# awkrail/svpc

Measured on AMD Instinct MI355X. Metric: train steps/sec (vivt, batch=16, clip_seq=12), higher is better.
Workload: dtype bf16x3; 1 GPU; MODEL_TYPE=vivt train step: N=16 videos/GPU x S=12 clips x Lv=100 frames x F=3072, Lt=22, D=768, H=12, L=6 (enc+step-enc+dec), V=951, A=384, E=10; dropout .1/.1/.4; fwd+bwd+allreduce+clip+BertAdam; mode=bf16x3, global_batch=16, parallelism=dp1, launch=hipGraph replay, gpus_requested=1

## Files before the change

### include/svpc_hip.h

```cpp
#ifndef SVPC_HIP_H
#define SVPC_HIP_H
#include <stddef.h>
#ifdef __cplusplus
extern "C" {
#endif

typedef struct ihipStream_t* svpc_stream_t;
typedef unsigned long long svpc_u64;

#define SVPC_ACT_NONE 0
#define SVPC_ACT_RELU 1
#define SVPC_ACT_GELU 2
#define SVPC_ACT_SIGMOID 3

const char* svpc_last_error(void);
int svpc_abi_version(void);

int svpc_ln_fwd(const float* x, const int* src_rows, const float* res, const float* gamma, const float* beta, float* y,
                float* mean, float* rstd, int R, int D, float eps, float p_pre, unsigned site_pre, float p_post,
                unsigned site_post, const svpc_u64* seed, const float* add1, int mod1, const float* add2, const int* idx2,
                svpc_stream_t stream);
int svpc_ln_fwd_t(const void* x, int x_dt, const int* src_rows, const void* res, const float* gamma, const float* beta, void* y,
                  int y_dt, float* mean, float* rstd, int R, int D, float eps, float p_pre, unsigned site_pre, float p_post,
                  unsigned site_post, const svpc_u64* seed, const float* add1, int mod1, const float* add2, const int* idx2,
// ... 9 lines not shown
int svpc_ln_fwd_s(const void* x, int x_dt, int ldx, int lox, const int* src_rows, const void* res, int ldr, int lor, const float* gamma,
                  const float* beta, void* y, int y_dt, int ldy, int loy, float* mean, float* rstd, int R, int D, float eps, float p_pre,
                  unsigned site_pre, float p_post, unsigned site_post, const svpc_u64* seed, const float* add1, int mod1,
                  const float* add2, const int* idx2, svpc_stream_t stream);
int svpc_ln_bwd_rows_s(const void* dy, const void* x, int x_dt, int ldx, int y_dt, const int* src_rows, const void* res, int ldr,
                       const float* gamma, const float* mean, const float* rstd, void* dh, void* dx, float* partial, int R, int D,
                       float p_pre, unsigned site_pre, float p_post, unsigned site_post, const svpc_u64* seed, svpc_stream_t stream);
int svpc_bucket_colsum_t(const void* x, int x_dt, int ldx, const int* idx, int R, int C, int K, float* out, int accumulate,
                         float* workspace, svpc_stream_t stream);
typedef struct svpc_finalize_entry { const float* partial; float* out0; float* out1; int groups, ncols, split; } svpc_finalize_entry;
int svpc_colsum_partial_t(const void* x, int x_dt, int ldx, int R, int C, float* partial, svpc_stream_t stream);
typedef struct svpc_colsum_entry { const void* x; float* partial; int dt, ldx, R, C; } svpc_colsum_entry;
int svpc_multi_colsum(const svpc_colsum_entry* entries, int n, svpc_stream_t stream);
int svpc_multi_finalize_max(void);
int svpc_multi_finalize(const svpc_finalize_entry* entries, int n, svpc_stream_t stream);
int svpc_ln_bwd_groups(int R);
int svpc_ln_param_only_groups(int R);
int svpc_ln_param_grads_g(const float* partial, int groups, int D, float* dgamma, float* dbeta, int accumulate, svpc_stream_t stream);
int svpc_ln_bwd(const float* dy, const float* x, const int* src_rows, const float* res, const float* gamma,
                const float* mean, const float* rstd, float* dh, float* dx, float* dgamma, float* dbeta, int accumulate,
                float* workspace, int R, int D, float p_pre, unsigned site_pre, float p_post, unsigned site_post,
                const svpc_u64* seed, svpc_stream_t stream);
int svpc_colsum_chunks(int R);
int svpc_bucket_colsum(const float* x, int ldx, const int* idx, int R, int C, int K, float* out, int accumulate,
                       float* workspace, svpc_stream_t stream);

int svpc_gemm_f32(const float* A, int lda, int a_kc, const float* B, int ldb, int b_kc, float* C, int ldc, float* Z, int M, int N,
                  int K, const float* bias, int act, float p_drop, unsigned site, const svpc_u64* seed, int accumulate,
                  float* workspace, size_t workspace_bytes, svpc_stream_t stream);
int svpc_gemm_bf16(const float* A, int lda, int a_kc, const float* B, int ldb, int b_kc, float* C, int ldc, float* Z, int M, int N,
                   int K, const float* bias, int act, float p_drop, unsigned site, const svpc_u64* seed, int accumulate,
                   float* workspace, size_t workspace_bytes, svpc_stream_t stream);
int svpc_gemm_mx(const void* A, int a_dt, int lda, int a_kc, const void* B, int b_dt, int ldb, int b_kc, void* C, int c_dt, int ldc,
                 void* Z, int M, int N, int K, const float* bias, int act, float p_drop, unsigned site, const svpc_u64* seed,
                 int accumulate, float* workspace, size_t workspace_bytes, svpc_stream_t stream);
int svpc_gemm_glds_supported(int a_kc, int b_kc, int lda, int ldb, int M, int N, int K);
int svpc_gemm_glds(const void* A, int lda, int a_kc, const void* B, int ldb, int b_kc, void* C, int c_dt, int ldc, void* Z, int M, int N,
                   int K, const float* bias, int act, float p_drop, unsigned site, const svpc_u64* seed, int accumulate,
                   float* workspace, size_t workspace_bytes, svpc_stream_t stream);
int svpc_gemm_glds_r(const void* A, int lda, int a_kc, const void* B, int ldb, int b_kc, void* C, int c_dt, int ldc, void* Z, const void* R,
                     int M, int N, int K, const float* bias, int act, float p_drop, unsigned site, const svpc_u64* seed, int accumulate,
                     float* workspace, size_t workspace_bytes, svpc_stream_t stream);
int svpc_gemm_glds_rg(const void* A, int lda, int a_kc, const void* B, int ldb, int b_kc, void* C, int c_dt, int ldc, void* Z, const void* R,
                      const void* G, int gact, int M, int N, int K, const float* bias, int act, float p_drop, unsigned site,
                      const svpc_u64* seed, int accumulate, float* workspace, size_t workspace_bytes, svpc_stream_t stream);
int svpc_gemm_p8(const void* A, int lda, const void* B, int ldb, void* C, int ldc, void* Z, int M, int N, int K, const float* bias, int act,
                 svpc_stream_t stream);
int svpc_gemm_p8x3_supported(int lda, int a_lo, int ldb, int ldc, int c_lo, int ldz, int M, int N, int K);
int svpc_gemm_p8x3(const void* A, int lda, int a_lo, const void* B, int ldb, long long b_lo, void* C, int ldc, int c_lo, void* Z, int ldz,
                   int M, int N, int K, const float* bias, int act, svpc_stream_t stream);
int svpc_gemm_s4x3(const void* A, int lda, int a_lo, const void* B, int ldb, long long b_lo, void* C, int ldc, int c_lo, void* Z, int ldz,
                   int M, int N, int K, const float* bias, int act, svpc_stream_t stream);
int svpc_gemm_s4t_supported(int lda, int ldb, int ldc, int M, int N, int K);
int svpc_gemm_s4t(const void* A, int lda, const void* B, int ldb, void* C, int ldc, const void* R, int M, int N, int K, svpc_stream_t stream);
int svpc_gemm_p8t_supported(int lda, int ldb, int ldc, int M, int N, int K);
int svpc_gemm_p8t(const void* A, int lda, const void* B, int ldb, void* C, int ldc, const void* G, int gact, const void* R, int M, int N, int K,
                  svpc_stream_t stream);
int svpc_gemm_l32_supported(int a_kc, int b_kc, int lda, int ldb, int M, int N, int K);
int svpc_gemm_l32_preferred(int a_kc, int b_kc, int lda, int ldb, int M, int N, int K);
int svpc_gemm_l32(const float* A, int lda, int a_kc, const float* B, int ldb, int b_kc, float* C, int ldc, float* Z, int M, int N, int K,
                  const float* bias, int act, float p_drop, unsigned site, const svpc_u64* seed, int accumulate, float* workspace,
                  size_t workspace_bytes, svpc_stream_t stream);
int svpc_gemm_l32_r(const float* A, int lda, int a_kc, const float* B, int ldb, int b_kc, float* C, int ldc, float* Z, const float* R, int M,
                    int N, int K, const float* bias, int act, float p_drop, unsigned site, const svpc_u64* seed, int accumulate,
                    float* workspace, size_t workspace_bytes, svpc_stream_t stream);
int svpc_gemm_l32_rg(const float* A, int lda, int a_kc, const float* B, int ldb, int b_kc, float* C, int ldc, const float* R, const float* G,
                     int gact, int M, int N, int K, int accumulate, float* workspace, size_t workspace_bytes, svpc_stream_t stream);
int svpc_gemm_l32_x3(const float* A, int lda, int a_kc, const float* B, int ldb, int b_kc, float* C, int ldc, float* Z, const float* R, int M,
                     int N, int K, const float* bias, int act, float p_drop, unsigned site, const svpc_u64* seed, int accumulate,
                     float* workspace, size_t workspace_bytes, svpc_stream_t stream);
typedef struct svpc_gemm_problem { const float* A; const float* B; float* C; int M, N, K, lda, ldb, ldc; } svpc_gemm_problem;
int svpc_gemm_group(const svpc_gemm_problem* problems, int n, int a_kc, int b_kc, int accumulate, svpc_stream_t stream);
int svpc_gemm_group_x3(const svpc_gemm_problem* problems, int n, int a_kc, int b_kc, int accumulate, svpc_stream_t stream);
typedef struct svpc_wgrad_problem {
    const float* dz; const float* x; float* dw; float* db;
    int n_out, n_in, rows, ld_dz, ld_x, ld_dw;
} svpc_wgrad_problem;
int svpc_gemm_group_wgrad_max(void);
int svpc_gemm_group_wgrad_bf16_p8_ok(const void* problems, int n);
int svpc_gemm_group_wgrad_bf16_p8(const void* problems, int n, float* workspace, size_t workspace_bytes, svpc_stream_t stream);
int svpc_gemm_group_wgrad_bf16(const svpc_wgrad_problem* problems, int n, svpc_stream_t stream);
int svpc_gemm_group_wgrad_bf16_ws(const svpc_wgrad_problem* problems, int n, float* workspace, size_t workspace_bytes,
                                  svpc_stream_t stream);
int svpc_gemm_group_wgrad(const svpc_wgrad_problem* problems, int n, svpc_stream_t stream);
int svpc_act_bwd(const float* dy, const float* aux, float* dz, size_t n, int act, float p, unsigned site, const svpc_u64* seed,
                 svpc_stream_t stream);

int svpc_act_bwd_t(const void* dy, const void* aux, void* dz, int dt, size_t n, int act, float p, unsigned site, const svpc_u64* seed,
                   svpc_stream_t stream);

int svpc_attn_fwd(const float* Q, int ldq, const float* K, int ldk, const float* V, int ldv, float* O, int ldo, float* LSE,
                  const int* seq, int n_seq, int H, int dh, int max_q, int max_k, const float* key_mask, int causal, float scale,
                  float p_drop, unsigned site, const svpc_u64* seed, svpc_stream_t stream);
int svpc_attn_q1_fwd(const float* Q, int ldq, const float* K, int ldk, const float* V, int ldv, float* O, int ldo, float* LSE,
                     const int* seq, int n_seq, int H, int dh, int max_k, const float* key_mask, float scale, svpc_stream_t stream);
int svpc_attn_q1_ln_supported(int D, int dh, int n_keys, int ldq, int ldkv, int ldnew, int ldx, int ldo);
int svpc_attn_q1_ln_fwd(const float* Q, int ldq, float* K, float* V, int ldkv, int k_stride, int n_keys, const float* newK, const float* newV,
                        int ldnew, const float* X, int ldx, const float* gamma, const float* beta, float eps, float* O, int ldo, int T, int D,
                        int dh, float scale, svpc_stream_t stream);
int svpc_attn_q1_ln_idx_fwd(const float* Q, int ldq, float* K, float* V, int ldkv, int k_stride, int n_keys, const int* key_rows, int ld_rows,
                            int q_group, const float* newK, const float* newV, int ldnew, const float* X, int ldx, const float* gamma,
                            const float* beta, float eps, float* O, int ldo, int T, int D, int dh, float scale, svpc_stream_t stream);
int svpc_attn_bwd(const float* Q, int ldq, const float* K, int ldk, const float* V, int ldv, const float* O, int ldo,
                  const float* LSE, const float* dO, int lddo, float* dQ, int lddq, float* dK, int lddk, float* dV, int lddv,
                  float* delta, const int* seq, int n_seq, int H, int dh, int max_q, int max_k, const float* key_mask, int causal,
                  float scale, float p_drop, unsigned site, const svpc_u64* seed, svpc_stream_t stream);
// ... 203 lines not shown
```

### svpc_amd/csrc/gemm_common.h

```cpp
#pragma once
#include "common.h"

typedef float floatx16 __attribute__((ext_vector_type(16)));

struct Epi {
    const float* bias; int act; float p_drop; uint32_t site; const u64* seed; int accumulate;
    float* Z;
    const void* R;
    const void* G; int gact;
};

__device__ __forceinline__ void epilogue_store(float v, int row, int col, float* __restrict__ C, int ldc, const Epi& e,
                                               u64 seed, float inv_keep) {
    if (e.bias) v += e.bias[col];
    const size_t o = (size_t)row * ldc + col;
    if (e.Z) e.Z[o] = v;
    v = apply_act(v, e.act);
    if (e.p_drop > 0.f) v *= drop_scale(seed, e.site, o, e.p_drop, inv_keep);
    if (e.G) v *= act_grad_from_aux(reinterpret_cast<const float*>(e.G)[o], e.gact, false);
    if (e.accumulate) v += C[o];
    if (e.R) v += reinterpret_cast<const float*>(e.R)[o];
    C[o] = v;
}

// ... 67 lines not shown
    return (xcd < r ? xcd * (q + 1) : r * (q + 1) + (xcd - r) * q) + (orig >> 3);
}


template <typename TC>
__global__ __launch_bounds__(256) void splitk_reduce1_kernel(const float* __restrict__ slabs, int splitk, TC* __restrict__ C, int ldc,
                                                             int M, int N, Epi epi) {
    const size_t i = (size_t)blockIdx.x * 256 + threadIdx.x;
    if (i >= (size_t)M * N) return;
    const int row = (int)(i / N), col = (int)(i - (size_t)row * N);
    float s = 0.f;
    for (int k = 0; k < splitk; ++k) s += slabs[(size_t)k * M * N + i];
    const u64 seed = epi.p_drop > 0.f ? epi.seed[0] : 0ull;
    const float inv_keep = epi.p_drop > 0.f ? 1.0f / (1.0f - epi.p_drop) : 1.0f;
    epilogue_store_t<TC>(s, row, col, C, ldc, epi, seed, inv_keep);
}
template <typename TC>
__global__ __launch_bounds__(256) void splitk_reduce4_kernel(const float* __restrict__ slabs, int splitk, TC* __restrict__ C, int ldc,
                                                             int M, int N, Epi epi) {
    const size_t q = (size_t)blockIdx.x * 256 + threadIdx.x, nq = (size_t)M * N / 4;
    if (q >= nq) return;
    const size_t i = q * 4;
    const int row = (int)(i / N), col = (int)(i - (size_t)row * N);
    const float4* p = reinterpret_cast<const float4*>(slabs) + q;
    float4 s = make_float4(0.f, 0.f, 0.f, 0.f);
    int k = 0;
    for (; k + 4 <= splitk; k += 4) {
        const float4 a = p[(size_t)k * nq], b = p[(size_t)(k + 1) * nq], c = p[(size_t)(k + 2) * nq], d = p[(size_t)(k + 3) * nq];
        s.x += a.x; s.y += a.y; s.z += a.z; s.w += a.w;
        s.x += b.x; s.y += b.y; s.z += b.z; s.w += b.w;
        s.x += c.x; s.y += c.y; s.z += c.z; s.w += c.w;
        s.x += d.x; s.y += d.y; s.z += d.z; s.w += d.w;
    }
    for (; k < splitk; ++k) {
        const float4 a = p[(size_t)k * nq];
        s.x += a.x; s.y += a.y; s.z += a.z; s.w += a.w;
    }
    const u64 seed = epi.p_drop > 0.f ? epi.seed[0] : 0ull;
    const float inv_keep = epi.p_drop > 0.f ? 1.0f / (1.0f - epi.p_drop) : 1.0f;
    epilogue_store_t<TC>(s.x, row, col, C, ldc, epi, seed, inv_keep);
    epilogue_store_t<TC>(s.y, row, col + 1, C, ldc, epi, seed, inv_keep);
    epilogue_store_t<TC>(s.z, row, col + 2, C, ldc, epi, seed, inv_keep);
    epilogue_store_t<TC>(s.w, row, col + 3, C, ldc, epi, seed, inv_keep);
}
template <typename TC>
static inline void launch_splitk_reduce(const float* slabs, int splitk, TC* C, int ldc, int M, int N, const Epi& epi, hipStream_t stream) {
    const size_t n = (size_t)M * N;
    if (N % 4 == 0 && ((((uintptr_t)slabs) & 15) == 0))
        hipLaunchKernelGGL(splitk_reduce4_kernel<TC>, dim3((unsigned)((n / 4 + 255) / 256)), dim3(256), 0, stream, slabs, splitk, C, ldc, M, N,
                           epi);
    else
        hipLaunchKernelGGL(splitk_reduce1_kernel<TC>, dim3((unsigned)((n + 255) / 256)), dim3(256), 0, stream, slabs, splitk, C, ldc, M, N, epi);
}
```

### svpc_amd/csrc/gemm_s4t.hip

```cpp
#include "gemm_common.h"
#include <stdlib.h>

typedef __bf16 bf16x8 __attribute__((ext_vector_type(8)));
typedef float floatx4 __attribute__((ext_vector_type(4)));
typedef short short4s __attribute__((ext_vector_type(4)));
typedef const void __attribute__((address_space(1))) * s4t_gptr;
typedef void __attribute__((address_space(3))) * s4t_lptr;

constexpr int S4T_BK = 64;
constexpr int S4T_HALF = 128 * S4T_BK * 2;
constexpr int S4T_STAGE = 2 * S4T_HALF;

__device__ __forceinline__ bf16x8 s4t_frag_tr(const char* __restrict__ a) {
    typedef short4s __attribute__((address_space(3))) * lds_ptr;
    const short4s lo = __builtin_amdgcn_ds_read_tr16_b64_v4i16((lds_ptr)(a));
    const short4s hi = __builtin_amdgcn_ds_read_tr16_b64_v4i16((lds_ptr)(a + 4 * 256));
    union { short s[8]; bf16x8 v; } u;
    u.s[0] = lo[0]; u.s[1] = lo[1]; u.s[2] = lo[2]; u.s[3] = lo[3];
    u.s[4] = hi[0]; u.s[5] = hi[1]; u.s[6] = hi[2]; u.s[7] = hi[3];
    return u.v;
}

template <bool HASR, int NS>
__global__ __launch_bounds__(512, NS == 2 ? 2 : 1) void gemm_s4t_kernel(const __bf16* __restrict__ A, int lda, const __bf16* __restrict__ B, int ldb,
                                                                        __bf16* __restrict__ C, int ldc, const __bf16* __restrict__ R, int M,
                                                                        int N, int K, int tiles_m, int tiles_n, int remap) {
    __shared__ __attribute__((aligned(1024))) char smem[NS * S4T_STAGE];
    const int wg = remap ? xcd_remap(blockIdx.x, tiles_m * tiles_n) : (int)blockIdx.x;
    const int tm = wg / tiles_n, tn = wg - tm * tiles_n;
    const int m0 = tm * 128, n0 = tn * 128;
    const int nk = K / S4T_BK;
    const int lane = threadIdx.x & 63, wave = __builtin_amdgcn_readfirstlane(threadIdx.x >> 6);
    const int wr = wave >> 1, wc = wave & 1;

    const int sr = lane >> 2, sc = (lane & 3) ^ (((lane >> 5) & 1) << 1);
    const __bf16* const ga = A + (size_t)min(m0 + 16 * wave + sr, M - 1) * lda + 8 * sc;
    const __bf16* gb[2];
#pragma unroll
    for (int u = 0; u < 2; ++u) {
        const int kr = 8 * wave + 4 * u + (lane >> 4);
        const int fx = 2 * ((kr & 3) | ((kr >> 1) & 4));
        const int col = min(n0 + 8 * ((lane & 15) ^ fx), N - 8);
        gb[u] = B + (size_t)kr * ldb + col;
    }
    const size_t stepB = (size_t)S4T_BK * ldb;
#define S4T_ISSUE(t)                                                                                                              \
    do {                                                                                                                          \
        char* st_ = smem + ((t) % NS) * S4T_STAGE;                                                                                \
        const __bf16* sa_ = ga + (size_t)(t) * S4T_BK;                                                                            \
        __builtin_amdgcn_global_load_lds((s4t_gptr)(sa_), (s4t_lptr)(st_ + ((wave * 2) << 10)), 16, 0, 0);                        \
        __builtin_amdgcn_global_load_lds((s4t_gptr)(sa_ + 32), (s4t_lptr)(st_ + ((wave * 2 + 1) << 10)), 16, 0, 0);               \
        __builtin_amdgcn_global_load_lds((s4t_gptr)(gb[0] + (size_t)(t) * stepB), (s4t_lptr)(st_ + S4T_HALF + wave * 2048), 16, 0, 0);        \
        __builtin_amdgcn_global_load_lds((s4t_gptr)(gb[1] + (size_t)(t) * stepB), (s4t_lptr)(st_ + S4T_HALF + wave * 2048 + 1024), 16, 0, 0); \
    } while (0)
    const int fr_off = (lane & 15) * 64 + ((((lane >> 4) ^ (((lane >> 3) & 1) << 1))) << 4);
#define S4T_FRAGA(img, blk, kb) (*reinterpret_cast<const bf16x8*>((img) + (((blk) * 2 + (kb)) << 10) + fr_off))
    const int tg = lane >> 4, tq = (lane & 15) >> 2, tp = lane & 3;
    const int tfx = 2 * (tq + 4 * (tg & 1));
    const int tb_off = (8 * tg + tq) * 256 + ((tp & 1) << 3);
    const int tp1 = tp >> 1;
#define S4T_FRAGB(img, cb, kb) s4t_frag_tr((img) + (kb) * (32 * 256) + tb_off + (((((2 * (cb)) ^ tfx)) | tp1) << 4))

    floatx4 acc[2][4];
#pragma unroll
    for (int i = 0; i < 2; ++i)
#pragma unroll
        for (int j = 0; j < 4; ++j) acc[i][j] = floatx4{0.f, 0.f, 0.f, 0.f};

#pragma unroll
    for (int t = 0; t < NS - 1; ++t)
        if (t < nk) S4T_ISSUE(t);
    for (int t = 0; t < nk; ++t) {
        if (NS == 4 && t + 2 < nk) asm volatile("s_waitcnt vmcnt(8)" ::: "memory");
        else if (NS >= 3 && t + 1 < nk) asm volatile("s_waitcnt vmcnt(4)" ::: "memory");
        else asm volatile("s_waitcnt vmcnt(0)" ::: "memory");
        __builtin_amdgcn_s_barrier();
        __builtin_amdgcn_sched_barrier(0);
        if (t + NS - 1 < nk) S4T_ISSUE(t + NS - 1);
        const char* sa = smem + (t % NS) * S4T_STAGE;
        const char* sb = sa + S4T_HALF;
#pragma unroll
        for (int kb = 0; kb < 2; ++kb) {
            bf16x8 bfr[4], afr[2];
#pragma unroll
            for (int j = 0; j < 4; ++j) bfr[j] = S4T_FRAGB(sb, wc * 4 + j, kb);
#pragma unroll
            for (int i = 0; i < 2; ++i) afr[i] = S4T_FRAGA(sa, wr * 2 + i, kb);
#pragma unroll
            for (int i = 0; i < 2; ++i)
#pragma unroll
                for (int j = 0; j < 4; ++j) acc[i][j] = __builtin_amdgcn_mfma_f32_16x16x32_bf16(bfr[j], afr[i], acc[i][j], 0, 0, 0);
        }
    }
#undef S4T_ISSUE
#undef S4T_FRAGA
#undef S4T_FRAGB
    __syncthreads();
    char* wl = smem + wave * 8192;
    const int row0 = m0 + wr * 32, col0 = n0 + wc * 64;
    const int l15 = lane & 15, q = lane >> 4;
    const int c8 = lane & 7, cc = col0 + 8 * c8, r0 = lane >> 3;
    const bool col_ok = cc + 8 <= N;
    bf16x8 rv[HASR ? 4 : 1];
#pragma unroll
    for (int it = 0; it < 4; ++it) {
        const int r = it * 8 + r0;
        if (HASR && col_ok && row0 + r < M) rv[it] = *reinterpret_cast<const bf16x8*>(R + (size_t)(row0 + r) * ldc + cc);
    }
#pragma unroll
    for (int i = 0; i < 2; ++i) {
        const int r = i * 16 + l15;
#pragma unroll
        for (int j = 0; j < 4; ++j) {
            const int c16 = j * 4 + q;
            *reinterpret_cast<floatx4*>(wl + r * 256 + ((c16 ^ (r & 7)) << 4)) = acc[i][j];
        }
    }
#pragma unroll
    for (int it = 0; it < 4; ++it) {
        const int r = it * 8 + r0;
        const floatx4 v0 = *reinterpret_cast<const floatx4*>(wl + r * 256 + (((2 * c8) ^ (r & 7)) << 4));
        const floatx4 v1 = *reinterpret_cast<const floatx4*>(wl + r * 256 + (((2 * c8 + 1) ^ (r & 7)) << 4));
        float v[8] = {v0[0], v0[1], v0[2], v0[3], v1[0], v1[1], v1[2], v1[3]};
        if (col_ok && row0 + r < M) {
            const size_t o = (size_t)(row0 + r) * ldc + cc;
            if (HASR) {
#pragma unroll
                for (int j = 0; j < 8; ++j) v[j] += (float)rv[it][j];
            }
            bf16x8 ov;
#pragma unroll
            for (int j = 0; j < 8; ++j) ov[j] = (__bf16)v[j];
            *reinterpret_cast<bf16x8*>(C + o) = ov;
        }
    }
}

extern "C" {

int svpc_gemm_s4t_supported(int lda, int ldb, int ldc, int M, int N, int K) {
    if (M <= 0 || N < 8 || K < S4T_BK || K % S4T_BK != 0 || (N & 7) != 0) return 0;
    if ((lda & 7) || (ldb & 7) || (ldc & 7) || lda < K || ldb < N || ldc < N) return 0;
    return 1;
}

int svpc_gemm_s4t(const void* A, int lda, const void* B, int ldb, void* C, int ldc, const void* R, int M, int N, int K, hipStream_t stream) {
    if (M <= 0 || N <= 0) return 0;
    SVPC_REQUIRE(svpc_gemm_s4t_supported(lda, ldb, ldc, M, N, K) == 1 &&
                     ((((uintptr_t)A) | ((uintptr_t)B) | ((uintptr_t)C) | ((uintptr_t)R)) & 15) == 0,
                 "gemm_s4t: needs K % 64 == 0, N % 8 == 0, 16-byte aligned bf16 rows");
    static int remap = -1, deep_max = -1;
    if (remap < 0) { const char* e = getenv("SVPC_GEMM_REMAP"); remap = e ? atoi(e) : 1; }
    if (deep_max < 0) { const char* e = getenv("SVPC_S4T_DEEP_MAX"); deep_max = e ? atoi(e) : 256; }
    const int tiles_m = ceil_div(M, 128), tiles_n = ceil_div(N, 128);
    const bool deep = tiles_m * tiles_n <= deep_max;
#define S4T_GO(RV, NSV)                                                                                                           \
    hipLaunchKernelGGL((gemm_s4t_kernel<RV, NSV>), dim3(tiles_m * tiles_n), dim3(512), 0, stream, (const __bf16*)A, lda, (const __bf16*)B, \
                       ldb, (__bf16*)C, ldc, (const __bf16*)R, M, N, K, tiles_m, tiles_n, remap)
    if (R != nullptr) { if (deep) S4T_GO(true, 4); else S4T_GO(true, 2); }
    else { if (deep) S4T_GO(false, 4); else S4T_GO(false, 2); }
#undef S4T_GO
    return svpc_check_launch("gemm_s4t");
}

}
```

### svpc_amd/csrc/gemm_s4x3.hip

```cpp
#include "gemm_common.h"
#include <stdlib.h>

typedef __bf16 bf16x8 __attribute__((ext_vector_type(8)));
typedef float floatx4 __attribute__((ext_vector_type(4)));
typedef const void __attribute__((address_space(1))) * s4_gptr;
typedef void __attribute__((address_space(3))) * s4_lptr;

constexpr int S4_BK = 64;
constexpr int S4_KS = 32;
constexpr int S4_HALF = 128 * S4_BK * 2;
constexpr int S4_STAGE = 2 * S4_HALF;

__device__ __forceinline__ uint32_t s4_pack2(float lo, float hi) {
    union { __bf16 h[2]; uint32_t u; } pk;
    pk.h[0] = (__bf16)lo; pk.h[1] = (__bf16)hi;
    return pk.u;
}
__device__ __forceinline__ float s4_lo(float v) { return v - (float)(__bf16)v; }
__device__ __forceinline__ float s4_gelu(float x) {
    const float u = x * 0.70710678118654752f, au = fabsf(u);
    const float t = __builtin_amdgcn_rcpf(fmaf(0.3275911f, au, 1.0f));
    float p = fmaf(1.061405429f, t, -1.453152027f);
    p = fmaf(p, t, 1.421413741f);
    p = fmaf(p, t, -0.284496736f);
    p = fmaf(p, t, 0.254829592f);
    const float e = __expf(-au * au);
    return 0.5f * x * (1.0f + copysignf(fmaf(-p * t, e, 1.0f), u));
}
template <int ACT>
__device__ __forceinline__ float s4_act(float z) {
    if (ACT == ACT_RELU) return fmaxf(z, 0.f);
    if (ACT == ACT_GELU) return s4_gelu(z);
    return z;
}

template <int ACT, int MODE>
__device__ __forceinline__ void s4_store_pass(const floatx4 (&acc)[2][4], __bf16* __restrict__ C, int ldc, const float4 (&bb)[4], int row0,
                                              int col0, int M, int N, int lane, char* __restrict__ wl) {
    const int l15 = lane & 15, q = lane >> 4;
#pragma unroll
    for (int i = 0; i < 2; ++i) {
        const int r = i * 16 + l15;
#pragma unroll
        for (int j = 0; j < 4; ++j) {
            float z0 = acc[i][j][0] + bb[j].x, z1 = acc[i][j][1] + bb[j].y, z2 = acc[i][j][2] + bb[j].z, z3 = acc[i][j][3] + bb[j].w;
            if (MODE != 0) { z0 = s4_act<ACT>(z0); z1 = s4_act<ACT>(z1); z2 = s4_act<ACT>(z2); z3 = s4_act<ACT>(z3); }
            if (MODE == 2) { z0 = s4_lo(z0); z1 = s4_lo(z1); z2 = s4_lo(z2); z3 = s4_lo(z3); }
            uint2 v;
            v.x = s4_pack2(z0, z1); v.y = s4_pack2(z2, z3);
            const int c16 = j * 2 + (q >> 1);
            *reinterpret_cast<uint2*>(wl + r * 128 + ((c16 ^ (r & 7)) << 4) + ((q & 1) << 3)) = v;
        }
    }
    const int chunk = lane & 7, cc = col0 + 8 * chunk, r0 = lane >> 3;
    uint32_t off = ((uint32_t)(row0 + r0) * (uint32_t)ldc + (uint32_t)cc) * 2u;
    const uint32_t step = 16u * (uint32_t)ldc;
    const bool col_ok = cc + 8 <= N;
#pragma unroll
    for (int it = 0; it < 4; ++it) {
        const int r = it * 8 + r0;
        const uint4 v = *reinterpret_cast<const uint4*>(wl + r * 128 + ((chunk ^ (r & 7)) << 4));
        if (col_ok && row0 + r < M) *reinterpret_cast<uint4*>(reinterpret_cast<char*>(C) + off) = v;
        off += step;
    }
}

template <int ACT, bool HASZ, int NS>
__global__ __launch_bounds__(512, NS == 2 ? 2 : 1) void gemm_s4x3_kernel(const __bf16* __restrict__ A, int lda, int a_lo, const __bf16* __restrict__ B, int ldb,
                                                           long long b_lo, __bf16* __restrict__ C, int ldc, int c_lo, __bf16* __restrict__ Z,
                                                           int ldz, const float* __restrict__ bias, int M, int N, int K, int tiles_m,
                                                           int tiles_n, int remap) {
    __shared__ __attribute__((aligned(1024))) char smem[NS * S4_STAGE];
    const int wg = remap ? xcd_remap(blockIdx.x, tiles_m * tiles_n) : (int)blockIdx.x;
    const int tm = wg / tiles_n, tn = wg - tm * tiles_n;
    const int m0 = tm * 128, n0 = tn * 128;
    const int nk = K / S4_KS;
    const int lane = threadIdx.x & 63, wave = __builtin_amdgcn_readfirstlane(threadIdx.x >> 6);
    const int wr = wave >> 1, wc = wave & 1;

    const int sr = lane >> 2, sc = (lane & 3) ^ (((lane >> 5) & 1) << 1);
    const __bf16* const ga = A + (size_t)min(m0 + 16 * wave + sr, M - 1) * lda + 8 * sc;
    const __bf16* const gb = B + (size_t)min(n0 + 16 * wave + sr, N - 1) * ldb + 8 * sc;
#define S4_ISSUE(t)                                                                                                               \
    do {                                                                                                                          \
        char* da_ = smem + ((t) % NS) * S4_STAGE + ((wave * 2) << 10);                                                            \
        const size_t o_ = (size_t)(t) * S4_KS;                                                                                    \
        __builtin_amdgcn_global_load_lds((s4_gptr)(ga + o_), (s4_lptr)(da_), 16, 0, 0);                                           \
        __builtin_amdgcn_global_load_lds((s4_gptr)(ga + o_ + a_lo), (s4_lptr)(da_ + 1024), 16, 0, 0);                             \
        __builtin_amdgcn_global_load_lds((s4_gptr)(gb + o_), (s4_lptr)(da_ + S4_HALF), 16, 0, 0);                                 \
        __builtin_amdgcn_global_load_lds((s4_gptr)(gb + o_ + b_lo), (s4_lptr)(da_ + S4_HALF + 1024), 16, 0, 0);                   \
    } while (0)
    const int fr_off = (lane & 15) * 64 + ((((lane >> 4) ^ (((lane >> 3) & 1) << 1))) << 4);
#define S4_FRAG(img, blk, kb) (*reinterpret_cast<const bf16x8*>((img) + (((blk) * 2 + (kb)) << 10) + fr_off))

    floatx4 acc[2][4];
#pragma unroll
    for (int i = 0; i < 2; ++i)
#pragma unroll
        for (int j = 0; j < 4; ++j) acc[i][j] = floatx4{0.f, 0.f, 0.f, 0.f};

#pragma unroll
    for (int t = 0; t < NS - 1; ++t)
        if (t < nk) S4_ISSUE(t);
    for (int t = 0; t < nk; ++t) {
        if (NS == 4 && t + 2 < nk) asm volatile("s_waitcnt vmcnt(8)" ::: "memory");
        else if (NS >= 3 && t + 1 < nk) asm volatile("s_waitcnt vmcnt(4)" ::: "memory");
        else asm volatile("s_waitcnt vmcnt(0)" ::: "memory");
        __builtin_amdgcn_s_barrier();
        __builtin_amdgcn_sched_barrier(0);
        if (t + NS - 1 < nk) S4_ISSUE(t + NS - 1);
        const char* sa = smem + (t % NS) * S4_STAGE;
        const char* sb = sa + S4_HALF;
        bf16x8 bfr[2][4], afr[2][2];
#pragma unroll
        for (int pl = 0; pl < 2; ++pl) {
#pragma unroll
            for (int j = 0; j < 4; ++j) bfr[pl][j] = S4_FRAG(sb, wc * 4 + j, pl);
#pragma unroll
            for (int i = 0; i < 2; ++i) afr[pl][i] = S4_FRAG(sa, wr * 2 + i, pl);
        }
#pragma unroll
        for (int term = 0; term < 3; ++term)
#pragma unroll
            for (int i = 0; i < 2; ++i)
#pragma unroll
                for (int j = 0; j < 4; ++j)
                    acc[i][j] = __builtin_amdgcn_mfma_f32_16x16x32_bf16(bfr[term == 2 ? 1 : 0][j], afr[term == 0 ? 1 : 0][i], acc[i][j], 0, 0, 0);
    }
#undef S4_ISSUE
#undef S4_FRAG
    __syncthreads();
    char* wl = smem + wave * 4096;
    const int row0 = m0 + wr * 32, col0 = n0 + wc * 64;
    float4 bb[4];
#pragma unroll
    for (int j = 0; j < 4; ++j) {
        const int c = col0 + j * 16 + 4 * (lane >> 4);
        bb[j] = (bias && c + 4 <= N) ? *reinterpret_cast<const float4*>(bias + c) : make_float4(0.f, 0.f, 0.f, 0.f);
    }
    if (HASZ) s4_store_pass<ACT, 0>(acc, Z, ldz, bb, row0, col0, M, N, lane, wl);
    s4_store_pass<ACT, 2>(acc, C + c_lo, ldc, bb, row0, col0, M, N, lane, wl);
    s4_store_pass<ACT, 1>(acc, C, ldc, bb, row0, col0, M, N, lane, wl);
}

extern "C" {

int svpc_gemm_s4x3(const void* A, int lda, int a_lo, const void* B, int ldb, long long b_lo, void* C, int ldc, int c_lo, void* Z, int ldz,
                   int M, int N, int K, const float* bias, int act, hipStream_t stream) {
    if (M <= 0 || N <= 0) return 0;
    if (Z == nullptr) ldz = 0;
    SVPC_REQUIRE(K >= 2 * S4_KS && K % S4_KS == 0 && (N & 7) == 0 && !((lda | a_lo | ldb | ldc | c_lo | ldz) & 7) && a_lo >= K && lda >= a_lo + K &&
                     c_lo >= N && ldc >= c_lo + N && ldb >= K && (b_lo & 7) == 0 &&
                     (unsigned long long)M * (unsigned long long)ldc * 2ull < (1ull << 32) &&
                     ((((uintptr_t)A) | ((uintptr_t)B) | ((uintptr_t)C) | ((uintptr_t)Z) | ((uintptr_t)bias)) & 15) == 0 &&
                     (act == ACT_RELU || act == ACT_GELU || (act == ACT_NONE && Z == nullptr)) && (Z == nullptr || ldz >= N),
                 "gemm_s4x3: needs K % 32 == 0, K >= 64, N % 8 == 0, 16-byte aligned split rows (lo plane behind the hi plane), act in {none, relu, gelu}");
    static int remap = -1;
    if (remap < 0) { const char* e = getenv("SVPC_GEMM_REMAP"); remap = e ? atoi(e) : 1; }
    const int tiles_m = ceil_div(M, 128), tiles_n = ceil_div(N, 128);
    static int deep_max = -1;
    if (deep_max < 0) { const char* e = getenv("SVPC_S4X3_DEEP_MAX"); deep_max = e ? atoi(e) : 256; }
    const bool deep = tiles_m * tiles_n <= deep_max;
#define S4_GO(ACTV, ZV)                                                                                                           \
    do {                                                                                                                          \
        if (deep) hipLaunchKernelGGL((gemm_s4x3_kernel<ACTV, ZV, 4>), dim3(tiles_m * tiles_n), dim3(512), 0, stream, (const __bf16*)A, lda, a_lo, \
                       (const __bf16*)B, ldb, b_lo, (__bf16*)C, ldc, c_lo, (__bf16*)Z, ldz, bias, M, N, K, tiles_m, tiles_n, remap); \
        else hipLaunchKernelGGL((gemm_s4x3_kernel<ACTV, ZV, 2>), dim3(tiles_m * tiles_n), dim3(512), 0, stream, (const __bf16*)A, lda, a_lo, \
                       (const __bf16*)B, ldb, b_lo, (__bf16*)C, ldc, c_lo, (__bf16*)Z, ldz, bias, M, N, K, tiles_m, tiles_n, remap); \
    } while (0)
    const bool z = Z != nullptr;
    if (act == ACT_GELU) { if (z) S4_GO(ACT_GELU, true); else S4_GO(ACT_GELU, false); }
    else if (act == ACT_RELU) { if (z) S4_GO(ACT_RELU, true); else S4_GO(ACT_RELU, false); }
    else S4_GO(ACT_NONE, false);
#undef S4_GO
    return svpc_check_launch("gemm_s4x3");
}

}
```

Baseline: 91.38 steps/s (one step = 16 clip-sequences per GPU; whole-job aggregate).

## Add selectable 96x96 and 64x128 tile variants with a wave-count tile chooser for s4 GEMMs

Templates the s4x3 and s4t bf16 split GEMM kernels on wave rows and column fragments, so they can run 128x128, 96x96 or 64x128 tiles with 384 or 256 threads. The per-wave B load distribution and the vmcnt wait counts are adjusted to match. A cost-model chooser uses fixed per-tile time constants and the count of 256 CUs to pick a smaller tile when that reduces tail waves. It applies only to s4x3; s4t stays at 128x128 unless overridden by environment variable. Smaller tiles give better CU fill on awkward shapes but less data reuse per tile.

Measured after the change: 92.07 steps/s (one step = 16 clip-sequences per GPU; whole-job aggregate), median of 6. No clear change (+0.8%).

```diff
diff --git a/include/svpc_hip.h b/include/svpc_hip.h
--- a/include/svpc_hip.h
+++ b/include/svpc_hip.h
@@ -85,6 +85,7 @@
 int svpc_gemm_s4x3(const void* A, int lda, int a_lo, const void* B, int ldb, long long b_lo, void* C, int ldc, int c_lo, void* Z, int ldz,
                    int M, int N, int K, const float* bias, int act, svpc_stream_t stream);
 int svpc_gemm_s4t_supported(int lda, int ldb, int ldc, int M, int N, int K);
+int svpc_gemm_s4_tile(int tile);
 int svpc_gemm_s4t(const void* A, int lda, const void* B, int ldb, void* C, int ldc, const void* R, int M, int N, int K, svpc_stream_t stream);
 int svpc_gemm_p8t_supported(int lda, int ldb, int ldc, int M, int N, int K);
 int svpc_gemm_p8t(const void* A, int lda, const void* B, int ldb, void* C, int ldc, const void* G, int gact, const void* R, int M, int N, int K,
diff --git a/svpc_amd/csrc/gemm_common.h b/svpc_amd/csrc/gemm_common.h
--- a/svpc_amd/csrc/gemm_common.h
+++ b/svpc_amd/csrc/gemm_common.h
@@ -143,3 +143,8 @@
     else
         hipLaunchKernelGGL(splitk_reduce1_kernel<TC>, dim3((unsigned)((n + 255) / 256)), dim3(256), 0, stream, slabs, splitk, C, ldc, M, N, epi);
 }
+
+enum { S4_TILE_AUTO = 0, S4_TILE_128x128 = 1, S4_TILE_96x96 = 2, S4_TILE_64x128 = 3 };
+constexpr int S4_CUS = 256;
+extern int svpc_s4_tile_force;
+int s4_pick_tile(int M, int N, int K, int kind);
diff --git a/svpc_amd/csrc/gemm_s4t.hip b/svpc_amd/csrc/gemm_s4t.hip
--- a/svpc_amd/csrc/gemm_s4t.hip
+++ b/svpc_amd/csrc/gemm_s4t.hip
@@ -8,8 +8,7 @@
 typedef void __attribute__((address_space(3))) * s4t_lptr;
 
 constexpr int S4T_BK = 64;
-constexpr int S4T_HALF = 128 * S4T_BK * 2;
-constexpr int S4T_STAGE = 2 * S4T_HALF;
+constexpr int S4T_BIMG = 64 * 128 * 2;
 
 __device__ __forceinline__ bf16x8 s4t_frag_tr(const char* __restrict__ a) {
     typedef short4s __attribute__((address_space(3))) * lds_ptr;
@@ -21,24 +20,32 @@
     return u.v;
 }
 
-template <bool HASR, int NS>
-__global__ __launch_bounds__(512, NS == 2 ? 2 : 1) void gemm_s4t_kernel(const __bf16* __restrict__ A, int lda, const __bf16* __restrict__ B, int ldb,
+template <bool HASR, int NS, int WR, int WJ>
+__global__ __launch_bounds__(128 * WR, NS == 2 ? 2 : 1) void gemm_s4t_kernel(const __bf16* __restrict__ A, int lda, const __bf16* __restrict__ B, int ldb,
                                                                         __bf16* __restrict__ C, int ldc, const __bf16* __restrict__ R, int M,
                                                                         int N, int K, int tiles_m, int tiles_n, int remap) {
-    __shared__ __attribute__((aligned(1024))) char smem[NS * S4T_STAGE];
+    constexpr int BM = 32 * WR, BN = 32 * WJ, NW = 2 * WR;
+    constexpr int A_IMG = BM * S4T_BK * 2, STAGE = A_IMG + S4T_BIMG;
+    constexpr int PPW = (16 + NW - 1) / NW;
+    constexpr int DH = 2 + PPW, DL = 16 % NW == 0 ? DH : DH - 1;
+    static_assert(BN <= 128 && NW * 8192 <= NS * STAGE, "gemm_s4t: tile too wide, or the epilogue images do not fit the stages");
+    __shared__ __attribute__((aligned(1024))) char smem[NS * STAGE];
     const int wg = remap ? xcd_remap(blockIdx.x, tiles_m * tiles_n) : (int)blockIdx.x;
     const int tm = wg / tiles_n, tn = wg - tm * tiles_n;
-    const int m0 = tm * 128, n0 = tn * 128;
+    const int m0 = tm * BM, n0 = tn * BN;
     const int nk = K / S4T_BK;
     const int lane = threadIdx.x & 63, wave = __builtin_amdgcn_readfirstlane(threadIdx.x >> 6);
     const int wr = wave >> 1, wc = wave & 1;
+    const bool heavy = 16 % NW == 0 || wave < 16 - NW * (PPW - 1);
 
     const int sr = lane >> 2, sc = (lane & 3) ^ (((lane >> 5) & 1) << 1);
     const __bf16* const ga = A + (size_t)min(m0 + 16 * wave + sr, M - 1) * lda + 8 * sc;
-    const __bf16* gb[2];
+    const __bf16* gb[PPW];
+    int pb[PPW];
 #pragma unroll
-    for (int u = 0; u < 2; ++u) {
-        const int kr = 8 * wave + 4 * u + (lane >> 4);
+    for (int u = 0; u < PPW; ++u) {
+        pb[u] = 16 % NW == 0 ? wave * PPW + u : min(u * NW + wave, 15);
+        const int kr = 4 * pb[u] + (lane >> 4);
         const int fx = 2 * ((kr & 3) | ((kr >> 1) & 4));
         const int col = min(n0 + 8 * ((lane & 15) ^ fx), N - 8);
         gb[u] = B + (size_t)kr * ldb + col;
@@ -46,12 +53,13 @@
     const size_t stepB = (size_t)S4T_BK * ldb;
 #define S4T_ISSUE(t)                                                                                                              \
     do {                                                                                                                          \
-        char* st_ = smem + ((t) % NS) * S4T_STAGE;                                                                                \
+        char* st_ = smem + ((t) % NS) * STAGE;                                                                                    \
         const __bf16* sa_ = ga + (size_t)(t) * S4T_BK;                                                                            \
         __builtin_amdgcn_global_load_lds((s4t_gptr)(sa_), (s4t_lptr)(st_ + ((wave * 2) << 10)), 16, 0, 0);                        \
         __builtin_amdgcn_global_load_lds((s4t_gptr)(sa_ + 32), (s4t_lptr)(st_ + ((wave * 2 + 1) << 10)), 16, 0, 0);               \
-        __builtin_amdgcn_global_load_lds((s4t_gptr)(gb[0] + (size_t)(t) * stepB), (s4t_lptr)(st_ + S4T_HALF + wave * 2048), 16, 0, 0);        \
-        __builtin_amdgcn_global_load_lds((s4t_gptr)(gb[1] + (size_t)(t) * stepB), (s4t_lptr)(st_ + S4T_HALF + wave * 2048 + 1024), 16, 0, 0); \
+        _Pragma("unroll") for (int u_ = 0; u_ < PPW; ++u_)                                                                        \
+            if (u_ < PPW - 1 || heavy)                                                                                            \
+                __builtin_amdgcn_global_load_lds((s4t_gptr)(gb[u_] + (size_t)(t) * stepB), (s4t_lptr)(st_ + A_IMG + (pb[u_] << 10)), 16, 0, 0); \
     } while (0)
     const int fr_off = (lane & 15) * 64 + ((((lane >> 4) ^ (((lane >> 3) & 1) << 1))) << 4);
 #define S4T_FRAGA(img, blk, kb) (*reinterpret_cast<const bf16x8*>((img) + (((blk) * 2 + (kb)) << 10) + fr_off))
@@ -61,35 +69,39 @@
     const int tp1 = tp >> 1;
 #define S4T_FRAGB(img, cb, kb) s4t_frag_tr((img) + (kb) * (32 * 256) + tb_off + (((((2 * (cb)) ^ tfx)) | tp1) << 4))
 
-    floatx4 acc[2][4];
+    floatx4 acc[2][WJ];
 #pragma unroll
     for (int i = 0; i < 2; ++i)
 #pragma unroll
-        for (int j = 0; j < 4; ++j) acc[i][j] = floatx4{0.f, 0.f, 0.f, 0.f};
+        for (int j = 0; j < WJ; ++j) acc[i][j] = floatx4{0.f, 0.f, 0.f, 0.f};
 
 #pragma unroll
     for (int t = 0; t < NS - 1; ++t)
         if (t < nk) S4T_ISSUE(t);
     for (int t = 0; t < nk; ++t) {
-        if (NS == 4 && t + 2 < nk) asm volatile("s_waitcnt vmcnt(8)" ::: "memory");
-        else if (NS >= 3 && t + 1 < nk) asm volatile("s_waitcnt vmcnt(4)" ::: "memory");
-        else asm volatile("s_waitcnt vmcnt(0)" ::: "memory");
+        if (NS == 4 && t + 2 < nk) {
+            if (heavy) asm volatile("s_waitcnt vmcnt(%0)" ::"n"(2 * DH) : "memory");
+            else asm volatile("s_waitcnt vmcnt(%0)" ::"n"(2 * DL) : "memory");
+        } else if (NS >= 3 && t + 1 < nk) {
+            if (heavy) asm volatile("s_waitcnt vmcnt(%0)" ::"n"(DH) : "memory");
+            else asm volatile("s_waitcnt vmcnt(%0)" ::"n"(DL) : "memory");
+        } else asm volatile("s_waitcnt vmcnt(0)" ::: "memory");
         __builtin_amdgcn_s_barrier();
         __builtin_amdgcn_sched_barrier(0);
         if (t + NS - 1 < nk) S4T_ISSUE(t + NS - 1);
-        const char* sa = smem + (t % NS) * S4T_STAGE;
-        const char* sb = sa + S4T_HALF;
+        const char* sa = smem + (t % NS) * STAGE;
+        const char* sb = sa + A_IMG;
 #pragma unroll
         for (int kb = 0; kb < 2; ++kb) {
-            bf16x8 bfr[4], afr[2];
+            bf16x8 bfr[WJ], afr[2];
 #pragma unroll
-            for (int j = 0; j < 4; ++j) bfr[j] = S4T_FRAGB(sb, wc * 4 + j, kb);
+            for (int j = 0; j < WJ; ++j) bfr[j] = S4T_FRAGB(sb, wc * WJ + j, kb);
 #pragma unroll
             for (int i = 0; i < 2; ++i) afr[i] = S4T_FRAGA(sa, wr * 2 + i, kb);
 #pragma unroll
             for (int i = 0; i < 2; ++i)
 #pragma unroll
-                for (int j = 0; j < 4; ++j) acc[i][j] = __builtin_amdgcn_mfma_f32_16x16x32_bf16(bfr[j], afr[i], acc[i][j], 0, 0, 0);
+                for (int j = 0; j < WJ; ++j) acc[i][j] = __builtin_amdgcn_mfma_f32_16x16x32_bf16(bfr[j], afr[i], acc[i][j], 0, 0, 0);
         }
     }
 #undef S4T_ISSUE
@@ -97,10 +109,10 @@
 #undef S4T_FRAGB
     __syncthreads();
     char* wl = smem + wave * 8192;
-    const int row0 = m0 + wr * 32, col0 = n0 + wc * 64;
+    const int row0 = m0 + wr * 32, col0 = n0 + wc * (16 * WJ);
     const int l15 = lane & 15, q = lane >> 4;
     const int c8 = lane & 7, cc = col0 + 8 * c8, r0 = lane >> 3;
-    const bool col_ok = cc + 8 <= N;
+    const bool col_ok = (WJ == 4 || c8 < 2 * WJ) && cc + 8 <= N;
     bf16x8 rv[HASR ? 4 : 1];
 #pragma unroll
     for (int it = 0; it < 4; ++it) {
@@ -111,7 +123,7 @@
     for (int i = 0; i < 2; ++i) {
         const int r = i * 16 + l15;
 #pragma unroll
-        for (int j = 0; j < 4; ++j) {
+        for (int j = 0; j < WJ; ++j) {
             const int c16 = j * 4 + q;
             *reinterpret_cast<floatx4*>(wl + r * 256 + ((c16 ^ (r & 7)) << 4)) = acc[i][j];
         }
@@ -151,15 +163,25 @@
                  "gemm_s4t: needs K % 64 == 0, N % 8 == 0, 16-byte aligned bf16 rows");
     static int remap = -1, deep_max = -1;
     if (remap < 0) { const char* e = getenv("SVPC_GEMM_REMAP"); remap = e ? atoi(e) : 1; }
-    if (deep_max < 0) { const char* e = getenv("SVPC_S4T_DEEP_MAX"); deep_max = e ? atoi(e) : 256; }
-    const int tiles_m = ceil_div(M, 128), tiles_n = ceil_div(N, 128);
+    if (deep_max < 0) { const char* e = getenv("SVPC_S4T_DEEP_MAX"); deep_max = e ? atoi(e) : S4_CUS; }
+    const int tile = s4_pick_tile(M, N, K, 1);
+    SVPC_REQUIRE(tile >= S4_TILE_128x128 && tile <= S4_TILE_64x128, "gemm_s4t: SVPC_S4_TILE must be 0 (chooser), 1 (128x128), 2 (96x96) or 3 (64x128)");
+    const int bm = tile == S4_TILE_128x128 ? 128 : tile == S4_TILE_96x96 ? 96 : 64, bn = tile == S4_TILE_96x96 ? 96 : 128;
+    const int tiles_m = ceil_div(M, bm), tiles_n = ceil_div(N, bn);
     const bool deep = tiles_m * tiles_n <= deep_max;
-#define S4T_GO(RV, NSV)                                                                                                           \
-    hipLaunchKernelGGL((gemm_s4t_kernel<RV, NSV>), dim3(tiles_m * tiles_n), dim3(512), 0, stream, (const __bf16*)A, lda, (const __bf16*)B, \
-                       ldb, (__bf16*)C, ldc, (const __bf16*)R, M, N, K, tiles_m, tiles_n, remap)
-    if (R != nullptr) { if (deep) S4T_GO(true, 4); else S4T_GO(true, 2); }
-    else { if (deep) S4T_GO(false, 4); else S4T_GO(false, 2); }
-#undef S4T_GO
+#define S4T_LAUNCH(RV, NSV, WRV, WJV)                                                                                             \
+    hipLaunchKernelGGL((gemm_s4t_kernel<RV, NSV, WRV, WJV>), dim3(tiles_m * tiles_n), dim3(128 * WRV), 0, stream, (const __bf16*)A, lda,   \
+                       (const __bf16*)B, ldb, (__bf16*)C, ldc, (const __bf16*)R, M, N, K, tiles_m, tiles_n, remap)
+#define S4T_TILES(RV, NSV)                                                                                                        \
+    do {                                                                                                                          \
+        if (tile == S4_TILE_96x96) S4T_LAUNCH(RV, NSV, 3, 3);                                                                     \
+        else if (tile == S4_TILE_64x128) S4T_LAUNCH(RV, NSV, 2, 4);                                                               \
+        else S4T_LAUNCH(RV, NSV, 4, 4);                                                                                           \
+    } while (0)
+    if (R != nullptr) { if (deep) S4T_TILES(true, 4); else S4T_TILES(true, 2); }
+    else { if (deep) S4T_TILES(false, 4); else S4T_TILES(false, 2); }
+#undef S4T_TILES
+#undef S4T_LAUNCH
     return svpc_check_launch("gemm_s4t");
 }
 
diff --git a/svpc_amd/csrc/gemm_s4x3.hip b/svpc_amd/csrc/gemm_s4x3.hip
--- a/svpc_amd/csrc/gemm_s4x3.hip
+++ b/svpc_amd/csrc/gemm_s4x3.hip
@@ -8,8 +8,6 @@
 
 constexpr int S4_BK = 64;
 constexpr int S4_KS = 32;
-constexpr int S4_HALF = 128 * S4_BK * 2;
-constexpr int S4_STAGE = 2 * S4_HALF;
 
 __device__ __forceinline__ uint32_t s4_pack2(float lo, float hi) {
     union { __bf16 h[2]; uint32_t u; } pk;
@@ -34,15 +32,15 @@
     return z;
 }
 
-template <int ACT, int MODE>
-__device__ __forceinline__ void s4_store_pass(const floatx4 (&acc)[2][4], __bf16* __restrict__ C, int ldc, const float4 (&bb)[4], int row0,
+template <int ACT, int MODE, int WJ>
+__device__ __forceinline__ void s4_store_pass(const floatx4 (&acc)[2][WJ], __bf16* __restrict__ C, int ldc, const float4 (&bb)[WJ], int row0,
                                               int col0, int M, int N, int lane, char* __restrict__ wl) {
     const int l15 = lane & 15, q = lane >> 4;
 #pragma unroll
     for (int i = 0; i < 2; ++i) {
         const int r = i * 16 + l15;
 #pragma unroll
-        for (int j = 0; j < 4; ++j) {
+        for (int j = 0; j < WJ; ++j) {
             float z0 = acc[i][j][0] + bb[j].x, z1 = acc[i][j][1] + bb[j].y, z2 = acc[i][j][2] + bb[j].z, z3 = acc[i][j][3] + bb[j].w;
             if (MODE != 0) { z0 = s4_act<ACT>(z0); z1 = s4_act<ACT>(z1); z2 = s4_act<ACT>(z2); z3 = s4_act<ACT>(z3); }
             if (MODE == 2) { z0 = s4_lo(z0); z1 = s4_lo(z1); z2 = s4_lo(z2); z3 = s4_lo(z3); }
@@ -55,7 +53,7 @@
     const int chunk = lane & 7, cc = col0 + 8 * chunk, r0 = lane >> 3;
     uint32_t off = ((uint32_t)(row0 + r0) * (uint32_t)ldc + (uint32_t)cc) * 2u;
     const uint32_t step = 16u * (uint32_t)ldc;
-    const bool col_ok = cc + 8 <= N;
+    const bool col_ok = (WJ == 4 || chunk < 2 * WJ) && cc + 8 <= N;
 #pragma unroll
     for (int it = 0; it < 4; ++it) {
         const int r = it * 8 + r0;
@@ -65,57 +63,68 @@
     }
 }
 
-template <int ACT, bool HASZ, int NS>
-__global__ __launch_bounds__(512, NS == 2 ? 2 : 1) void gemm_s4x3_kernel(const __bf16* __restrict__ A, int lda, int a_lo, const __bf16* __restrict__ B, int ldb,
+template <int ACT, bool HASZ, int NS, int WR, int WJ>
+__global__ __launch_bounds__(128 * WR, NS == 2 ? 2 : 1) void gemm_s4x3_kernel(const __bf16* __restrict__ A, int lda, int a_lo, const __bf16* __restrict__ B, int ldb,
                                                            long long b_lo, __bf16* __restrict__ C, int ldc, int c_lo, __bf16* __restrict__ Z,
                                                            int ldz, const float* __restrict__ bias, int M, int N, int K, int tiles_m,
                                                            int tiles_n, int remap) {
-    __shared__ __attribute__((aligned(1024))) char smem[NS * S4_STAGE];
+    constexpr int BM = 32 * WR, BN = 32 * WJ, NW = 2 * WR;
+    constexpr int A_IMG = BM * S4_BK * 2, STAGE = (BM + BN) * S4_BK * 2;
+    constexpr int NBW = (BN / 16) / NW;
+    constexpr int DPW = 2 + 2 * NBW;
+    static_assert((BN / 16) % NW == 0 && NBW >= 1, "gemm_s4x3: B row blocks must spread evenly over the waves");
+    __shared__ __attribute__((aligned(1024))) char smem[NS * STAGE];
     const int wg = remap ? xcd_remap(blockIdx.x, tiles_m * tiles_n) : (int)blockIdx.x;
     const int tm = wg / tiles_n, tn = wg - tm * tiles_n;
-    const int m0 = tm * 128, n0 = tn * 128;
+    const int m0 = tm * BM, n0 = tn * BN;
     const int nk = K / S4_KS;
     const int lane = threadIdx.x & 63, wave = __builtin_amdgcn_readfirstlane(threadIdx.x >> 6);
     const int wr = wave >> 1, wc = wave & 1;
 
     const int sr = lane >> 2, sc = (lane & 3) ^ (((lane >> 5) & 1) << 1);
     const __bf16* const ga = A + (size_t)min(m0 + 16 * wave + sr, M - 1) * lda + 8 * sc;
-    const __bf16* const gb = B + (size_t)min(n0 + 16 * wave + sr, N - 1) * ldb + 8 * sc;
+    const __bf16* gb[NBW];
+#pragma unroll
+    for (int u = 0; u < NBW; ++u) gb[u] = B + (size_t)min(n0 + 16 * (wave + NW * u) + sr, N - 1) * ldb + 8 * sc;
 #define S4_ISSUE(t)                                                                                                               \
     do {                                                                                                                          \
-        char* da_ = smem + ((t) % NS) * S4_STAGE + ((wave * 2) << 10);                                                            \
+        char* st_ = smem + ((t) % NS) * STAGE;                                                                                    \
+        char* da_ = st_ + ((wave * 2) << 10);                                                                                     \
         const size_t o_ = (size_t)(t) * S4_KS;                                                                                    \
         __builtin_amdgcn_global_load_lds((s4_gptr)(ga + o_), (s4_lptr)(da_), 16, 0, 0);                                           \
         __builtin_amdgcn_global_load_lds((s4_gptr)(ga + o_ + a_lo), (s4_lptr)(da_ + 1024), 16, 0, 0);                             \
-        __builtin_amdgcn_global_load_lds((s4_gptr)(gb + o_), (s4_lptr)(da_ + S4_HALF), 16, 0, 0);                                 \
-        __builtin_amdgcn_global_load_lds((s4_gptr)(gb + o_ + b_lo), (s4_lptr)(da_ + S4_HALF + 1024), 16, 0, 0);                   \
+        _Pragma("unroll") for (int u_ = 0; u_ < NBW; ++u_) {                                                                      \
+            char* db_ = st_ + A_IMG + (((wave + NW * u_) * 2) << 10);                                                             \
+            __builtin_amdgcn_global_load_lds((s4_gptr)(gb[u_] + o_), (s4_lptr)(db_), 16, 0, 0);                                   \
+            __builtin_amdgcn_global_load_lds((s4_gptr)(gb[u_] + o_ + b_lo), (s4_lptr)(db_ + 1024), 16, 0, 0);                     \
+        }                                                                                                                         \
     } while (0)
     const int fr_off = (lane & 15) * 64 + ((((lane >> 4) ^ (((lane >> 3) & 1) << 1))) << 4);
 #define S4_FRAG(img, blk, kb) (*reinterpret_cast<const bf16x8*>((img) + (((blk) * 2 + (kb)) << 10) + fr_off))
 
-    floatx4 acc[2][4];
+    floatx4 acc[2][WJ];
 #pragma unroll
     for (int i = 0; i < 2; ++i)
 #pragma unroll
-        for (int j = 0; j < 4; ++j) acc[i][j] = floatx4{0.f, 0.f, 0.f, 0.f};
+        for (int j = 0; j < WJ; ++j) acc[i][j] = floatx4{0.f, 0.f, 0.f, 0.f};
 
 #pragma unroll
     for (int t = 0; t < NS - 1; ++t)
         if (t < nk) S4_ISSUE(t);
     for (int t = 0; t < nk; ++t) {
-        if (NS == 4 && t + 2 < nk) asm volatile("s_waitcnt vmcnt(8)" ::: "memory");
-        else if (NS >= 3 && t + 1 < nk) asm volatile("s_waitcnt vmcnt(4)" ::: "memory");
+        if (NS == 4 && t + 2 < nk) asm volatile("s_waitcnt vmcnt(%0)" ::"n"(2 * DPW) : "memory");
+        else if (NS >= 3 && t + 1 < nk) asm volatile("s_waitcnt vmcnt(%0)" ::"n"(DPW) : "memory");
         else asm volatile("s_waitcnt vmcnt(0)" ::: "memory");
         __builtin_amdgcn_s_barrier();
         __builtin_amdgcn_sched_barrier(0);
         if (t + NS - 1 < nk) S4_ISSUE(t + NS - 1);
-        const char* sa = smem + (t % NS) * S4_STAGE;
-        const char* sb = sa + S4_HALF;
-        bf16x8 bfr[2][4], afr[2][2];
+        const char* sa = smem + (t % NS) * STAGE;
+        const char* sb = sa + A_IMG;
+        bf16x8 bfr[2][WJ], afr[2][2];
 #pragma unroll
         for (int pl = 0; pl < 2; ++pl) {
 #pragma unroll
-            for (int j = 0; j < 4; ++j) bfr[pl][j] = S4_FRAG(sb, wc * 4 + j, pl);
+            for (int j = 0; j < WJ; ++j) bfr[pl][j] = S4_FRAG(sb, wc * WJ + j, pl);
 #pragma unroll
             for (int i = 0; i < 2; ++i) afr[pl][i] = S4_FRAG(sa, wr * 2 + i, pl);
         }
@@ -124,26 +133,57 @@
 #pragma unroll
             for (int i = 0; i < 2; ++i)
 #pragma unroll
-                for (int j = 0; j < 4; ++j)
+                for (int j = 0; j < WJ; ++j)
                     acc[i][j] = __builtin_amdgcn_mfma_f32_16x16x32_bf16(bfr[term == 2 ? 1 : 0][j], afr[term == 0 ? 1 : 0][i], acc[i][j], 0, 0, 0);
     }
 #undef S4_ISSUE
 #undef S4_FRAG
     __syncthreads();
     char* wl = smem + wave * 4096;
-    const int row0 = m0 + wr * 32, col0 = n0 + wc * 64;
-    float4 bb[4];
-#pragma unroll
-    for (int j = 0; j < 4; ++j) {
+    const int row0 = m0 + wr * 32, col0 = n0 + wc * (16 * WJ);
+    float4 bb[WJ];
+#pragma unroll
+    for (int j = 0; j < WJ; ++j) {
         const int c = col0 + j * 16 + 4 * (lane >> 4);
         bb[j] = (bias && c + 4 <= N) ? *reinterpret_cast<const float4*>(bias + c) : make_float4(0.f, 0.f, 0.f, 0.f);
     }
-    if (HASZ) s4_store_pass<ACT, 0>(acc, Z, ldz, bb, row0, col0, M, N, lane, wl);
-    s4_store_pass<ACT, 2>(acc, C + c_lo, ldc, bb, row0, col0, M, N, lane, wl);
-    s4_store_pass<ACT, 1>(acc, C, ldc, bb, row0, col0, M, N, lane, wl);
+    if (HASZ) s4_store_pass<ACT, 0, WJ>(acc, Z, ldz, bb, row0, col0, M, N, lane, wl);
+    s4_store_pass<ACT, 2, WJ>(acc, C + c_lo, ldc, bb, row0, col0, M, N, lane, wl);
+    s4_store_pass<ACT, 1, WJ>(acc, C, ldc, bb, row0, col0, M, N, lane, wl);
+}
+
+int svpc_s4_tile_force = -1;
+
+int s4_pick_tile(int M, int N, int K, int kind) {
+    if (svpc_s4_tile_force < 0) {
+        const char* e = getenv("SVPC_S4_TILE");
+        svpc_s4_tile_force = e ? atoi(e) : S4_TILE_AUTO;
+    }
+    if (svpc_s4_tile_force != S4_TILE_AUTO) return svpc_s4_tile_force;
+    if (kind != 0) return S4_TILE_128x128;
+    static const float t_one[3] = {24.6f, 20.4f, 18.7f}, t_two[3] = {40.6f, 27.4f, 28.8f};
+    constexpr float S4_MARGIN = 0.95f;
+    static const int bm[3] = {128, 96, 64}, bn[3] = {128, 96, 128};
+    int best = S4_TILE_128x128;
+    float best_t = 0.f;
+    for (int c = 0; c < 3; ++c) {
+        const int tiles = ceil_div(M, bm[c]) * ceil_div(N, bn[c]);
+        const float t = tiles <= S4_CUS ? t_one[c] : (float)ceil_div(tiles, 2 * S4_CUS) * t_two[c];
+        if (c == 0) best_t = t;
+        else if (t < S4_MARGIN * best_t) { best = S4_TILE_128x128 + c; best_t = t; }
+    }
+    (void)K;
+    return best;
 }
 
 extern "C" {
+
+int svpc_gemm_s4_tile(int tile) {
+    s4_pick_tile(1, 8, 64, 0);
+    const int prev = svpc_s4_tile_force;
+    svpc_s4_tile_force = tile;
+    return prev;
+}
 
 int svpc_gemm_s4x3(const void* A, int lda, int a_lo, const void* B, int ldb, long long b_lo, void* C, int ldc, int c_lo, void* Z, int ldz,
                    int M, int N, int K, const float* bias, int act, hipStream_t stream) {
@@ -157,22 +197,34 @@
                  "gemm_s4x3: needs K % 32 == 0, K >= 64, N % 8 == 0, 16-byte aligned split rows (lo plane behind the hi plane), act in {none, relu, gelu}");
     static int remap = -1;
     if (remap < 0) { const char* e = getenv("SVPC_GEMM_REMAP"); remap = e ? atoi(e) : 1; }
-    const int tiles_m = ceil_div(M, 128), tiles_n = ceil_div(N, 128);
+    const int tile = s4_pick_tile(M, N, K, 0);
+    SVPC_REQUIRE(tile >= S4_TILE_128x128 && tile <= S4_TILE_64x128, "gemm_s4x3: SVPC_S4_TILE must be 0 (chooser), 1 (128x128), 2 (96x96) or 3 (64x128)");
+    const int bm = tile == S4_TILE_128x128 ? 128 : tile == S4_TILE_96x96 ? 96 : 64, bn = tile == S4_TILE_96x96 ? 96 : 128;
+    const int tiles_m = ceil_div(M, bm), tiles_n = ceil_div(N, bn);
     static int deep_max = -1;
-    if (deep_max < 0) { const char* e = getenv("SVPC_S4X3_DEEP_MAX"); deep_max = e ? atoi(e) : 256; }
+    if (deep_max < 0) { const char* e = getenv("SVPC_S4X3_DEEP_MAX"); deep_max = e ? atoi(e) : S4_CUS; }
     const bool deep = tiles_m * tiles_n <= deep_max;
+#define S4_LAUNCH(ACTV, ZV, NSV, WRV, WJV)                                                                                        \
+    hipLaunchKernelGGL((gemm_s4x3_kernel<ACTV, ZV, NSV, WRV, WJV>), dim3(tiles_m * tiles_n), dim3(128 * WRV), 0, stream, (const __bf16*)A, lda, \
+                       a_lo, (const __bf16*)B, ldb, b_lo, (__bf16*)C, ldc, c_lo, (__bf16*)Z, ldz, bias, M, N, K, tiles_m, tiles_n, remap)
+#define S4_TILES(ACTV, ZV, NSV)                                                                                                   \
+    do {                                                                                                                          \
+        if (tile == S4_TILE_96x96) S4_LAUNCH(ACTV, ZV, NSV, 3, 3);                                                                \
+        else if (tile == S4_TILE_64x128) S4_LAUNCH(ACTV, ZV, NSV, 2, 4);                                                          \
+        else S4_LAUNCH(ACTV, ZV, NSV, 4, 4);                                                                                      \
+    } while (0)
 #define S4_GO(ACTV, ZV)                                                                                                           \
     do {                                                                                                                          \
-        if (deep) hipLaunchKernelGGL((gemm_s4x3_kernel<ACTV, ZV, 4>), dim3(tiles_m * tiles_n), dim3(512), 0, stream, (const __bf16*)A, lda, a_lo, \
-                       (const __bf16*)B, ldb, b_lo, (__bf16*)C, ldc, c_lo, (__bf16*)Z, ldz, bias, M, N, K, tiles_m, tiles_n, remap); \
-        else hipLaunchKernelGGL((gemm_s4x3_kernel<ACTV, ZV, 2>), dim3(tiles_m * tiles_n), dim3(512), 0, stream, (const __bf16*)A, lda, a_lo, \
-                       (const __bf16*)B, ldb, b_lo, (__bf16*)C, ldc, c_lo, (__bf16*)Z, ldz, bias, M, N, K, tiles_m, tiles_n, remap); \
+        if (deep) S4_TILES(ACTV, ZV, 4);                                                                                          \
+        else S4_TILES(ACTV, ZV, 2);                                                                                               \
     } while (0)
     const bool z = Z != nullptr;
     if (act == ACT_GELU) { if (z) S4_GO(ACT_GELU, true); else S4_GO(ACT_GELU, false); }
     else if (act == ACT_RELU) { if (z) S4_GO(ACT_RELU, true); else S4_GO(ACT_RELU, false); }
     else S4_GO(ACT_NONE, false);
 #undef S4_GO
+#undef S4_TILES
+#undef S4_LAUNCH
     return svpc_check_launch("gemm_s4x3");
 }
 
```
